# google/bayesnf

Hardware: AMD Instinct MI355X
Metric: train-steps/sec x ensemble_size (member-steps/s, whole job) (higher is better)
Workload: dtype bf16; 1 GPU; C2 chickenpox-like MAP: N=10232 rows, D=3, F=57, width=512, depth=2, NORMAL, full batch, lr=0.005; members_per_gpu=64, ensemble_size=64, parallelism=ensemble-shard x1 (no data-path collective)

## Files before the change

bayesnf_amd/csrc/bnf_api.hip:

```cpp
#include <hip/hip_runtime.h>
#include <cstring>
#include <rocprim/device/device_radix_sort.hpp>
#include <rocprim/device/device_segmented_radix_sort.hpp>

#include <dlfcn.h>

#include <atomic>
#include <cmath>
#include <cstdarg>
#include <cstdio>
#include <cstdlib>
#include <cstring>
#include <string>
#include <vector>

#include "../../include/bnf.h"
#include "bnf_gemm.h"
#include "bnf_kernels.h"
#include "bnf_panel.h"
#include "bnf_gemm8.h"
#include "bnf_sampling.h"
#include "bnf_extremes.h"
#include "bnf_episodes.h"
#include "bnf_scoring.h"
#include "bnf_rps.h"
#include "bnf_totals.h"
#include "bnf_dependence.h"
#include "bnf_ranking.h"
#include "bnf_stacking.h"

using namespace bnf;

static thread_local char g_err[512] = "";
static int fail(int code, const char* fmt, ...) {
  va_list ap;
  va_start(ap, fmt);
  vsnprintf(g_err, sizeof(g_err), fmt, ap);
  va_end(ap);
  return code;
}
#define HIPCHK(expr)                                                                   \
  do {                                                                                 \
    hipError_t _e = (expr);                                                            \
    if (_e != hipSuccess)                                                              \
      return fail(BNF_ERR_HIP, "%s failed: %s (%s:%d)", #expr, hipGetErrorString(_e), \
                  __FILE__, __LINE__);                                                 \
  } while (0)

enum KernelId {
  KID_PACK = 0, KID_FEAT, KID_FWD0, KID_FWD, KID_ROWLOSS, KID_LASTBWD, KID_DGRAD, KID_DGRAD0,
  KID_FEATBWD, KID_WGRAD0, KID_WGRAD, KID_ADAM, KID_VISAMPLE, KID_VIADAM, KID_FWDLAST, KID_PANEL, KID_COUNT
};
static const char* kKernelNames[KID_COUNT] = {
    "pack_weights", "featurize", "gemm_fwd_l0", "gemm_fwd", "row_loss", "last_bwd", "gemm_dgrad",
    "gemm_dgrad0", "feat_bwd", "gemm_wgrad_l0", "gemm_wgrad", "adam_map", "vi_sample", "vi_adam",
    "gemm_fwd_last", "panel_fwd_bwd"};

struct TimedLaunch {
  int kid;
  hipEvent_t t0, t1;
};

static constexpr int64_t kAtPad = 128;

struct bnf_handle {
  bnf_config cfg;
  NetDev nd;
  FreqTab ft;
  bool bf16 = false;
  int f32_split = 0;
  bool q8 = false;
  bool c8 = false;
  uint8_t* Wf8[BNF_MAX_LAYERS] = {}; uint8_t* Wb8[BNF_MAX_LAYERS] = {};
  uint8_t* H0q = nullptr;
  float* qscale = nullptr;
  int es = 4;
  int Ev = 0;
  int S = 1;
  int L = 0, W = 0, F = 0, Fp = 0, P = 0;
  int Wt = 0;
  bool pad = false;
  int64_t Pf = 0, Pp = 0;
  float* gradf = nullptr;
  float* theta_pad = nullptr;
  int32_t* pad_src = nullptr;
  int32_t* fold_src = nullptr;
  std::vector<int32_t> pad_src_h, fold_src_h;
  int32_t* fbmeta = nullptr;
  std::vector<int32_t> fbmeta_h;
  int fb_in_group = -1;
  int64_t N = 0, B = 0, Bp = 0;
  hipStream_t stream = nullptr;
  hipStream_t stream2 = nullptr;
  hipEvent_t ev_dz[BNF_MAX_LAYERS] = {};
  hipEvent_t ev_wg = nullptr;
  bool overlap = false;
  bool bound = false;
  int64_t adam_t = 0;
  float* params = nullptr;
  float* state = nullptr;
  char* ws = nullptr;
  const float* X = nullptr;
  const float* y = nullptr;
  float* theta_c = nullptr;
  float* grad = nullptr;
  float* stab = nullptr;
  float* stab_pred = nullptr;
  void* H0 = nullptr; void* H0t = nullptr;
  const float* ext_eps = nullptr;
  const uint32_t* vi_keys = nullptr; int64_t vi_key_rows = 0, vi_key_t0 = 0;
  const uint32_t* vi_draw_keys = nullptr; int64_t vi_draw_rows = 0;
  const int32_t* row_tab = nullptr; int64_t row_tab_epochs = 0, row_tab_e0 = 0;
  const uint32_t* row_keys = nullptr; int64_t row_keys_epochs = 0, row_keys_e0 = 0; int32_t row_key_rounds = 0;
  uint32_t* perm_bits[2] = {nullptr, nullptr}; int32_t* perm_val[2] = {nullptr, nullptr};
  unsigned* perm_seg = nullptr; void* perm_tmp = nullptr; size_t perm_tmp_bytes = 0;
  bool perm_ready = false;
  size_t owned_bytes = 0;
  int32_t* perm = nullptr; int64_t perm_epoch = -1;
  int32_t* leaf_off = nullptr; uint8_t* leaf_id = nullptr; int32_t n_leaves = 0;
  bool adam_clear_all = false;
  bool h0l = false;
  bool fold0 = false;
  void* A[BNF_MAX_LAYERS]; void* H[BNF_MAX_LAYERS]; void* Ht[BNF_MAX_LAYERS];
  void* dZ[BNF_MAX_LAYERS]; void* dZt[BNF_MAX_LAYERS];
  void* Kn[BNF_MAX_LAYERS]; void* Kt[BNF_MAX_LAYERS];
  int64_t pack_batch[BNF_MAX_LAYERS];
  float* dH0 = nullptr; float* out = nullptr; float* ybat = nullptr; float* loss_raw = nullptr;
  float* vacc = nullptr; float* dv = nullptr;
  bool vi_sample_pack = true, vi_keep_z = false;
  bool panel = false;
  void* Wf[BNF_MAX_LAYERS]; void* Wb[BNF_MAX_LAYERS];
  void* park[BNF_MAX_LAYERS];
    unsigned long long* prof_buf = nullptr;
  double prof_gap[16] = {0, 0, 0, 0, 0, 0, 0, 0, 0, 0, 0, 0, 0, 0, 0, 0};
  double prof_blocks = 0;
  int prof_threads = 0;
  bool recompute_a0 = false;
  bool fuse_last = false;
  int num_cus = 256;
  int tn_ring = 1;
  int skinny = 1;
  int big_tiles = 1;
  float* scal = nullptr;
  StepState* step_state = nullptr;
  hipGraphExec_t graph_exec = nullptr;
  int64_t graph_cols = 0;
  float* graph_losses = nullptr;
  int graph_mode = 0;
  float* qscratch = nullptr;
// ... 674 lines not shown
template <typename T>
static void run_pack_fragments(bnf_handle* h, const float* theta, int nmem) {
  LaunchScope ls(h, KID_PACK);
  int tiles = 0;
  const PackJobs jb = pack_jobs(h, &tiles);
  hipLaunchKernelGGL((k_pack_layers<T>), dim3((unsigned)tiles * (unsigned)nmem), dim3(256), 0, h->stream,
                     theta, (int64_t)h->Pf, jb, h->nd, h->scal);
}

template <int WN, int RT, bool H0L, bool DEEP, int CH, int FP, bool F0, bool C8 = false>
static void launch_panel_f(bnf_handle* h, const PanelArgs& pa) {
  constexpr int kLds = panel_lds_bytes(WN, RT, H0L, CH, FP);
  static_assert(kLds <= 160 * 1024, "LDS per workgroup");
  static std::atomic<uint64_t> attr_done{0};
  allow_lds(h, &k_panel_fwd_bwd<WN, RT, H0L, DEEP, CH, FP, F0, C8>, kLds, &attr_done);
  PanelArgs pa2 = pa;
  pa2.ablate = h->ablate;
  const unsigned blocks = (unsigned)(pa.members * pa.panels);
  {
    EpiArgs tmp{};
    phase_prof_begin(h, KID_PANEL, blocks, &tmp);
    pa2.prof = tmp.prof;
  }
  {
    LaunchScope ls(h, KID_PANEL);
    hipLaunchKernelGGL((k_panel_fwd_bwd<WN, RT, H0L, DEEP, CH, FP, F0, C8>), dim3(blocks), dim3(512), kLds, h->stream, pa2);
  }
  phase_prof_end(h, KID_PANEL, blocks, 512);
}
template <int WN, int RT, bool H0L, bool DEEP, int CH, int FP>
static void launch_panel_d(bnf_handle* h, const PanelArgs& pa) {
  if constexpr (H0L) {
    if (h->fold0) {
      if (pa.c8) {
        launch_panel_f<WN, RT, H0L, DEEP, CH, FP, true, true>(h, pa);
        return;
      }
      launch_panel_f<WN, RT, H0L, DEEP, CH, FP, true>(h, pa);
      return;
    }
  }
  launch_panel_f<WN, RT, H0L, DEEP, CH, FP, false>(h, pa);
}

template <int WN, int RT, bool H0L, int CH = 1, int FP = 64>
static void launch_panel(bnf_handle* h, const PanelArgs& pa) {
  if (pa.n_layers == 2) launch_panel_d<WN, RT, H0L, false, CH, FP>(h, pa);
  else launch_panel_d<WN, RT, H0L, true, CH, FP>(h, pa);
}

static void run_panel(bnf_handle* h, const float* theta, int nmem, const RowSrc& rs, float c,
                      const LossSink& sink, bool fragments_packed = false) {
  const int64_t Bp = h->Bp;
  if (!fragments_packed) run_pack_fragments<bf16_t>(h, theta, nmem);
  {
    LaunchScope ls(h, KID_FEAT);
    dim3 grid(cdiv(h->B, kFeatRows) * (unsigned)nmem);
    const size_t lds = (size_t)kFeatRows * (h->Fp + 8) * 2;
    static std::atomic<uint64_t> attr_done{0};
    allow_lds(h, &k_featurize<bf16_t>, 160 * 1024, &attr_done);
    hipLaunchKernelGGL((k_featurize<bf16_t>), grid, dim3(kFeatRows), lds, h->stream, h->nd, rs, h->X, h->stab,
                       h->y, h->scal, h->B, (bf16_t*)h->H0, Bp * h->Fp, (bf16_t*)h->H0t,
                       (int64_t)h->Fp * Bp, (int32_t)Bp, h->ybat, Bp, (int32_t)nmem, (int32_t)(h->fold0 ? 2 : 0), h->H0q);
  }
  bool feat_bwd_fused = false;
  PanelArgs pa{};
  pa.F = h->F; pa.Fp = h->Fp; pa.B = (int32_t)h->B; pa.members = nmem; pa.Wt = h->Wt;
  pa.theta = theta; pa.theta_stride = h->Pf; pa.scal = h->scal;
  const int L = h->L;
  pa.n_layers = L;
  for (int l = 0; l < L; ++l) {
    pa.off_bias[l] = h->nd.off_bias[l]; pa.off_ls[l] = h->nd.off_ls[l];
    pa.Wf[l] = (const bf16_t*)h->Wf[l]; pa.Wb[l] = (const bf16_t*)h->Wb[l];
    pa.Hout[l] = (bf16_t*)h->H[l]; pa.dZ[l] = (bf16_t*)h->dZ[l]; pa.park[l] = (bf16_t*)h->park[l];
  }
  pa.off_bias_out = h->nd.off_bias[L]; pa.off_ko = h->nd.off_kernel[L];
  pa.off_os = h->nd.off_os; pa.off_law = h->nd.off_law; pa.off_lns = h->nd.off_lns;
  pa.off_shape = h->nd.off_shape; pa.off_infl = h->nd.off_infl; pa.obs = h->nd.obs;
  pa.H0 = (const bf16_t*)h->H0t; pa.H0rm = (const bf16_t*)h->H0; pa.h0_batch = Bp * h->Fp;
  pa.w0_batch = h->pack_batch[0]; pa.w1_batch = h->pack_batch[1];
  pa.act_batch = Bp * h->W;
  pa.dH0t = h->dH0; pa.dh0_batch = (int64_t)h->Fp * Bp; pa.ldt = (int32_t)Bp;
  pa.ybat = h->ybat; pa.row_batch = Bp; pa.out = h->out; pa.out_batch = Bp;
  pa.grad = h->gradf; pa.grad_stride = h->Pf;
  pa.loss = sink.loss; pa.loss_raw = sink.raw; pa.loss_stride = sink.stride; pa.S = h->S;
  pa.loss_scale = sink.scale; pa.lik_c = c; pa.st = sink.st;
  pa.q8 = h->q8 ? 1 : 0; pa.qscale = h->qscale;
  pa.c8 = h->c8 ? 1 : 0; pa.w8_batch = (int64_t)h->W * h->W;
  for (int l = 0; l < L; ++l) { pa.Wf8[l] = h->Wf8[l]; pa.Wb8[l] = h->Wb8[l]; }
  auto with_fused_featbwd = [&]() {
    pa.fbmeta = h->fbmeta; pa.off_lsa = h->nd.off_lsa; pa.n_groups = h->nd.n_groups; pa.n_inputs = h->nd.D;
    pa.fb_in_group = h->fb_in_group;
    feat_bwd_fused = h->fbmeta != nullptr;
  };
  if (h->W == 1024) {
    pa.panels = (int32_t)(Bp / panel_rows(8, 2));
    if (h->h0l) {
      with_fused_featbwd();
      launch_panel<8, 2, true, 2>(h, pa);
    } else {
      launch_panel<8, 2, false, 2>(h, pa);
    }
  } else if (h->W == 512) {
    pa.panels = (int32_t)(Bp / panel_rows(8, 4));
    if (h->h0l) {
      with_fused_featbwd();
      launch_panel<8, 4, true>(h, pa);
    } else {
// ... 476 lines not shown
      return fail(BNF_ERR_INVALID, "fourier_degree[%d]", d);
    }
  }
  for (int k = 0; k < cfg->n_interact; ++k) {
    nd.interact[k][0] = cfg->interact[k][0];
    nd.interact[k][1] = cfg->interact[k][1];
  }
  nd.off_lns = cfg->off_log_noise_scale; nd.off_shape = cfg->off_shape; nd.off_infl = cfg->off_inflated;
  for (int l = 0; l <= h->L; ++l) {
    nd.off_bias[l] = cfg->off_bias[l];
    nd.off_kernel[l] = cfg->off_kernel[l];
  }
  h->Pf = h->P;
  if (h->pad) {
    const int W = h->W, Wt = h->Wt;
    int64_t pos = h->P;
    h->fold_src_h.resize((size_t)h->P);
    for (int64_t i = 0; i < h->P; ++i) h->fold_src_h[(size_t)i] = (int32_t)i;
    auto leaf = [&](int32_t off_true, int rows_t, int cols_t, int rows_p, int cols_p) {
      const int32_t off_pad = (int32_t)pos;
      for (int r = 0; r < rows_p; ++r)
        for (int c = 0; c < cols_p; ++c) {
          const bool in = r < rows_t && c < cols_t;
          const int32_t src = in ? off_true + r * cols_t + c : -1;
          h->pad_src_h.push_back(src);
          if (in) h->fold_src_h[(size_t)src] = (int32_t)pos;
          ++pos;
        }
      return off_pad;
    };
    for (int l = 0; l < h->L; ++l) {
      nd.off_bias[l] = leaf(cfg->off_bias[l], 1, Wt, 1, W);
      const int rt = (l == 0) ? h->F : Wt, rp = (l == 0) ? h->F : W;
      nd.off_kernel[l] = leaf(cfg->off_kernel[l], rt, Wt, rp, W);
    }
    nd.off_kernel[h->L] = leaf(cfg->off_kernel[h->L], Wt, 1, W, 1);
    while (pos % 4) { h->pad_src_h.push_back(-1); ++pos; }
    h->Pp = pos; h->Pf = pos;
  }
  for (int l = 0; l < h->L; ++l) nd.off_ls[l] = cfg->off_layer_scale[l];
  nd.off_os = cfg->off_output_scale; nd.off_lsa = cfg->off_lsa; nd.off_law = cfg->off_act_weight;
  h->ft.n = cfg->n_freqs;
  for (int j = 0; j < cfg->n_freqs; ++j) {
    h->ft.f[j] = cfg->freq[j];
    h->ft.h[j] = cfg->harmonic[j];
  }
  for (int k = 0; k < KID_COUNT; ++k) { h->acc_ms[k] = 0; h->acc_calls[k] = 0; }
  if (const char* ab = getenv("BNF_ABLATE")) h->ablate = atoi(ab);
  h->num_cus = prop.multiProcessorCount > 0 ? prop.multiProcessorCount : 256;
  if (const char* bt = getenv("BNF_BIG_TILES")) h->big_tiles = atoi(bt);
  if (const char* sk = getenv("BNF_WGRAD_SKINNY")) h->skinny = atoi(sk);
  if (const char* rg = getenv("BNF_TN_RING")) h->tn_ring = atoi(rg);
  if (const char* gm = getenv("BNF_GRAPH")) h->graph_mode = atoi(gm);
  h->adam_clear_all = getenv("BNF_ADAM_CLEAR_ALL") != nullptr;
  if (const char* v = getenv("BNF_VI_SAMPLE_PACK")) h->vi_sample_pack = atoi(v) != 0;
  if (const char* v = getenv("BNF_VI_KEEP_Z")) h->vi_keep_z = atoi(v) != 0;
  {
    int want = cfg->pipeline;
    if (const char* pf = getenv("BNF_PIPELINE")) want = atoi(pf);
    if (want != 0 && want != 1 && want != 3) {
      delete h;
      return fail(BNF_ERR_INVALID, "pipeline %d (0 auto, 1 layers, 3 panel)", want);
    }
    const bool can_panel = !cfg->forward_only && h->bf16 && h->L >= 2 && (h->W == 256 || h->W == 512 || h->W == 1024) && h->Fp <= 128;
    if (want == 3 && !can_panel) {
      delete h;
      return fail(BNF_ERR_INVALID, "panel pipeline needs a bf16 training handle with depth >= 2, width 256/512/1024 and <= 128 features");
    }
    h->panel = can_panel && (want == 3 || want == 0);
    if (h->q8 && !h->panel && !cfg->forward_only) {
      delete h;
      return fail(BNF_ERR_INVALID, "dtype fp8 (fp8 operand storage for the weight gradients) needs the row-panel pipeline: "
                  "depth >= 2, width 256 / 512 / 1024 after padding to 64, <= 128 padded features");
    }
    if (h->panel) h->Bp = align_up(h->B, 256);
    h->c8 = h->q8 && h->panel && !(getenv("BNF_FP8_CONTRACT") && atoi(getenv("BNF_FP8_CONTRACT")) == 0);
    const bool fl_ok = h->bf16 ? fused_last_supported<bf16_t>(h->W) : fused_last_supported<float>(h->W);
    h->fuse_last = !cfg->forward_only && !h->panel && want == 0 && fl_ok;
    h->recompute_a0 = !cfg->forward_only && !h->panel && want == 0 && h->L >= 2 && h->Fp <= 128;
  }
  h->h0l = panel_h0l(h);
  h->fold0 = h->h0l && h->F + 2 <= h->Fp && !(getenv("BNF_PANEL_FOLD0") && atoi(getenv("BNF_PANEL_FOLD0")) == 0);
  h->c8 = h->c8 && h->fold0;
  if (h->h0l &&
      !(getenv("BNF_PANEL_FEATBWD") && atoi(getenv("BNF_PANEL_FEATBWD")) == 0)) {
    int in_group = -1;
    for (int g = 0; g < cfg->n_groups; ++g)
      if (cfg->group_kind[g] == BNF_GROUP_INPUT) in_group = g;
    if (in_group >= 0) {
      std::vector<int32_t>& m = h->fbmeta_h;
      const int Fp = h->Fp;
      m.assign(Fp * 4 + BNF_MAX_GROUPS, 0);
      auto put = [&](int col, int kind, int g, int d1, int d2, int partner, int ucol, float coef) {
        m[4 * col] = kind | (g << 8) | (d1 << 16) | (d2 << 24);
        m[4 * col + 1] = partner | (ucol << 8);
        memcpy(&m[4 * col + 2], &coef, 4);
      };
      for (int c = 0; c < Fp; ++c) put(c, kFbNone, 0xff, 0xff, 0xff, 0, 0, 0.f);
      const int cin = cfg->group_col0[in_group];
      for (int g = 0; g < cfg->n_groups; ++g) {
        const int c0 = cfg->group_col0[g], nc = cfg->group_ncols[g];
        m[4 * Fp + g] = cfg->group_scale_off[g];
        switch (cfg->group_kind[g]) {
          case BNF_GROUP_INPUT:
            for (int d = 0; d < nc; ++d) put(c0 + d, kFbInput, g, d, 0xff, 0, 0, 0.f);
            break;
// ... 1292 lines not shown
```

bayesnf_amd/csrc/bnf_kernels.h:

```cpp
#pragma once

#include "bnf_device.h"
#include "../../include/bnf.h"

namespace bnf {

constexpr int kScalGroup = BNF_MAX_LAYERS + 2;
constexpr int kScalInput = kScalGroup + BNF_MAX_GROUPS;
constexpr int kScalGfac = kScalInput + BNF_MAX_INPUTS;
constexpr int kScalStride = kScalGfac + BNF_MAX_GROUPS;

__device__ __forceinline__ void sincos_rev(float x, float* s, float* c) {
  sincosf(6.28318530717958647692f * x, s, c);
}

struct NetDev {
  int32_t D, F, Fp, W, Wt, depth, P, n_groups, n_freqs, n_interact, obs;
  int32_t group_kind[BNF_MAX_GROUPS], group_arg[BNF_MAX_GROUPS], group_ncols[BNF_MAX_GROUPS],
      group_col0[BNF_MAX_GROUPS], group_scale_off[BNF_MAX_GROUPS];
  int32_t fdeg[BNF_MAX_INPUTS];
  float in_scale[BNF_MAX_INPUTS];
  int32_t interact[BNF_MAX_INTERACT][2];
  int32_t off_lns, off_shape, off_infl;
  int32_t off_bias[BNF_MAX_LAYERS + 1], off_kernel[BNF_MAX_LAYERS + 1], off_ls[BNF_MAX_LAYERS];
  int32_t off_os, off_lsa, off_law;
};

struct RowSrc {
  int32_t mode;
  int32_t S;
  uint64_t seed;
  uint64_t epoch;
  int64_t pos0;
  int64_t n_rows;
  int64_t member_offset;
  const int32_t* table;
  int64_t table_ld;
};

__device__ __forceinline__ int64_t row_of(const RowSrc& rs, int e, int64_t r) {
  if (rs.mode == 0) return r;
  if (rs.mode == 3) return (int64_t)rs.table[(int64_t)(e / rs.S) * rs.table_ld + rs.pos0 + r];
  if (rs.mode == 1) {
    const FeistelKey fk = feistel_key(rs.seed, (uint32_t)(rs.member_offset + e / rs.S), rs.epoch,
                                      STREAM_SHUFFLE, (uint64_t)rs.n_rows);
    return (int64_t)feistel_perm(fk, (uint64_t)(rs.pos0 + r));
  }
  const FeistelKey fk = feistel_key(rs.seed, 0u, rs.epoch, STREAM_VI_BATCH, (uint64_t)rs.n_rows);
  return (int64_t)feistel_perm(fk, (uint64_t)r);
}

constexpr float kTwoPiF = 6.2831854820251465f;

struct FreqTab {
  int32_t n;
  float f[BNF_MAX_FREQS], h[BNF_MAX_FREQS];
};

__global__ void k_seasonal_table(const float* __restrict__ X, int64_t n_rows, int D, FreqTab ft,
                                 float* __restrict__ S) {
  const int64_t r = (int64_t)blockIdx.x * blockDim.x + threadIdx.x;
  if (r >= n_rows) return;
  const float t = X[r * D];
  for (int j = 0; j < ft.n; ++j) {
    const float cf = kTwoPiF * ft.f[j];
    const float y = cf * t;
    double s, c;
    sincos((double)y, &s, &c);
    S[r * (2 * ft.n) + j] = (float)c / ft.h[j];
    S[r * (2 * ft.n) + ft.n + j] = (float)s / ft.h[j];
  }
}

constexpr int kFeatRows = 128;

template <typename T>
__global__ __launch_bounds__(kFeatRows) void k_featurize(
    NetDev nd, RowSrc rs, const float* __restrict__ X, const float* __restrict__ Stab,
    const float* __restrict__ y, const float* __restrict__ scal, int64_t B,
    T* __restrict__ H0, int64_t h0_batch, T* __restrict__ H0f, int64_t h0f_batch, int32_t ldt,
    float* __restrict__ ybat, int64_t ybat_batch, int32_t n_members, int32_t n_ones,
    uint8_t* __restrict__ H0q = nullptr) {
  extern __shared__ __attribute__((aligned(16))) char fsm[];
  constexpr int kEpc = 16 / Elem<T>::kBytes;
  T* tile = reinterpret_cast<T*>(fsm);
  const int pitch = nd.Fp + kEpc;
  const int e = (int)(blockIdx.x % (uint32_t)n_members);
  const int64_t r0 = (int64_t)(blockIdx.x / (uint32_t)n_members) * kFeatRows;
  const int64_t r = r0 + threadIdx.x;
  const float* sc = scal + (int64_t)e * kScalStride;
  if (r < B) {
    const int64_t row = row_of(rs, e, r);
    const float* x = X + row * nd.D;
    float xr[BNF_MAX_INPUTS], u[BNF_MAX_INPUTS];
#pragma unroll
    for (int d = 0; d < BNF_MAX_INPUTS; ++d) xr[d] = x[min(d, nd.D - 1)];
#pragma unroll
    for (int d = 0; d < BNF_MAX_INPUTS; ++d) u[d] = xr[d] / sc[kScalInput + min(d, nd.D - 1)];
    T* trow = tile + threadIdx.x * pitch;
    auto put = [&](int col, float v) { Elem<T>::store(trow + col, v); };
    for (int g = 0; g < nd.n_groups; ++g) {
      const float sp = sc[kScalGroup + g];
      const int c0 = nd.group_col0[g], nc = nd.group_ncols[g];
      const int kind = nd.group_kind[g];
      if (kind == BNF_GROUP_INPUT) {
        for (int d = 0; d < nd.D; ++d) put(c0 + d, u[d] * sp);
      } else if (kind == BNF_GROUP_FOURIER) {
        const int deg = nc >> 1;
        float ud = 0.f;
#pragma unroll
        for (int d = 0; d < BNF_MAX_INPUTS; ++d)
          if (d == nd.group_arg[g]) ud = u[d];
        for (int k = 0; k < deg; ++k) {
          float sn, cs;
          if constexpr (sizeof(T) == 2) {
            const float x = ud * (float)(1u << k);
            const float fx = x - floorf(x);
            sn = __builtin_amdgcn_sinf(fx);
            cs = __builtin_amdgcn_cosf(fx);
            const float q = __builtin_amdgcn_rcpf((float)(k + 1)) * sp;
            put(c0 + k, cs * q);
            put(c0 + deg + k, sn * q);
            continue;
          }
          sincos_rev(ud * (float)(1u << k), &sn, &cs);
          const float den = (float)(k + 1);
          put(c0 + k, (cs / den) * sp);
          put(c0 + deg + k, (sn / den) * sp);
        }
      } else if (kind == BNF_GROUP_SEASONAL) {
        const float* srow = Stab + row * nc;
        int j = 0;
        for (; j + 8 <= nc; j += 8) {
          float v[8];
#pragma unroll
          for (int q = 0; q < 8; ++q) v[q] = srow[j + q];
#pragma unroll
          for (int q = 0; q < 8; ++q) put(c0 + j + q, v[q] * sp);
        }
        for (; j < nc; ++j) put(c0 + j, srow[j] * sp);
      } else {
        for (int k = 0; k < nc; ++k) {
          float up = 0.f, uq = 0.f;
#pragma unroll
          for (int d = 0; d < BNF_MAX_INPUTS; ++d) {
            if (d == nd.interact[k][0]) up = u[d];
            if (d == nd.interact[k][1]) uq = u[d];
          }
          put(c0 + k, (up * uq) * sp);
        }
      }
    }
    for (int c = nd.F; c < nd.Fp; ++c) Elem<T>::store(trow + c, c < nd.F + n_ones ? 1.f : 0.f);
    if (ybat) ybat[(int64_t)e * ybat_batch + r] = y ? y[row] : 0.f;
  }
  __syncthreads();
  const int cpr = nd.Fp / kEpc;
  const int n_live = (int)min((int64_t)kFeatRows, B - r0);
  const int pitch_b = pitch * Elem<T>::kBytes;
  auto copy_out = [&](char* dst_block, int ppr, int sb, auto conv) {
    const int total = n_live * ppr;
    const int dc = kFeatRows % ppr, d_off = (kFeatRows / ppr) * pitch_b + dc * sb, wrap = pitch_b - ppr * sb;
    int cc = (int)threadIdx.x % ppr, off = ((int)threadIdx.x / ppr) * pitch_b + cc * sb;
    for (int q = threadIdx.x; q < total; q += 4 * kFeatRows) {
      u32x4 v[4];
      int offs[4];
#pragma unroll
      for (int i = 0; i < 4; ++i) {
        offs[i] = off;
        cc += dc; off += d_off;
        if (cc >= ppr) { cc -= ppr; off += wrap; }
      }
#pragma unroll
      for (int i = 0; i < 4; ++i)
        if (q + i * kFeatRows < total) v[i] = conv(fsm + offs[i]);
#pragma unroll
      for (int i = 0; i < 4; ++i)
        if (q + i * kFeatRows < total) *reinterpret_cast<u32x4*>(dst_block + (size_t)(q + i * kFeatRows) * 16) = v[i];
    }
  };
  if (n_live > 0) {
    copy_out(reinterpret_cast<char*>(H0 + (int64_t)e * h0_batch + r0 * nd.Fp), cpr, 16,
             [&](const char* src) { return *reinterpret_cast<const u32x4*>(src); });
  }
  if constexpr (sizeof(T) == 2) {
    if (H0q && n_live > 0) {
      __builtin_amdgcn_s_setreg(1 | (23 << 6), 1);
      copy_out(reinterpret_cast<char*>(H0q + (int64_t)e * h0_batch + r0 * nd.Fp), nd.Fp / 16, 32, [&](const char* src) {
        const u32x4 lo = *reinterpret_cast<const u32x4*>(src);
        const u32x4 hi = *reinterpret_cast<const u32x4*>(src + 16);
        return u32x4{bf16x4_to_fp8(lo[0], lo[1], 1.f), bf16x4_to_fp8(lo[2], lo[3], 1.f), bf16x4_to_fp8(hi[0], hi[1], 1.f),
                     bf16x4_to_fp8(hi[2], hi[3], 1.f)};
      });
    }
    if (H0f) {
      T* df = H0f + (int64_t)e * h0f_batch;
      const int ks0 = nd.Fp / 16;
      for (int q = threadIdx.x; q < kFeatRows * cpr; q += kFeatRows) {
        const int lr = q % kFeatRows, cc = q / kFeatRows;
        const int64_t rr = r0 + lr;
        if (rr < B)
          *reinterpret_cast<u32x4*>(df + ((((rr >> 5) * ks0 + (cc >> 1)) * 64 + (cc & 1) * 32 + (rr & 31)) << 3)) =
              *reinterpret_cast<const u32x4*>(tile + lr * pitch + cc * kEpc);
      }
    }
  }
  (void)ldt;
}

__global__ __launch_bounds__(256) void k_feat_bwd(
    NetDev nd, RowSrc rs, const float* __restrict__ X, const float* __restrict__ Stab,
    const float* __restrict__ theta, int64_t theta_stride, const float* __restrict__ scal, int64_t B,
    const float* __restrict__ dH0t, int64_t dh0_batch, int32_t ldt, float* __restrict__ grad,
    int64_t grad_stride) {
  __shared__ float red[4][BNF_MAX_GROUPS + BNF_MAX_INPUTS];
  const int e = blockIdx.y;
  const int64_t r = (int64_t)blockIdx.x * blockDim.x + threadIdx.x;
  const float* th = theta + (int64_t)e * theta_stride;
  const float* sc = scal + (int64_t)e * kScalStride;
  float dfs[BNF_MAX_GROUPS], dlsa[BNF_MAX_INPUTS];
#pragma unroll
  for (int g = 0; g < BNF_MAX_GROUPS; ++g) dfs[g] = 0.f;
#pragma unroll
  for (int d = 0; d < BNF_MAX_INPUTS; ++d) dlsa[d] = 0.f;
  if (r < B) {
    const int64_t row = row_of(rs, e, r);
    const float* x = X + row * nd.D;
    float xr[BNF_MAX_INPUTS], u[BNF_MAX_INPUTS], du[BNF_MAX_INPUTS];
#pragma unroll
    for (int d = 0; d < BNF_MAX_INPUTS; ++d) xr[d] = x[min(d, nd.D - 1)];
#pragma unroll
    for (int d = 0; d < BNF_MAX_INPUTS; ++d) {
      du[d] = 0.f;
      u[d] = d < nd.D ? xr[d] / sc[kScalInput + min(d, nd.D - 1)] : 0.f;
    }
    const float* dhp = dH0t + (int64_t)e * dh0_batch + r;
    auto dh = [&](int col) { return dhp[(int64_t)col * ldt]; };
#pragma unroll
    for (int g = 0; g < BNF_MAX_GROUPS; ++g) {
      if (g >= nd.n_groups) continue;
      const float sp = sc[kScalGroup + g];
      const int c0 = nd.group_col0[g], nc = nd.group_ncols[g];
      const int kind = nd.group_kind[g];
      float acc = 0.f;
      if (kind == BNF_GROUP_INPUT) {
#pragma unroll
        for (int d = 0; d < BNF_MAX_INPUTS; ++d)
          if (d < nd.D) {
            const float dhv = dh(c0 + d);
            acc += dhv * u[d];
            du[d] += sp * dhv;
          }
      } else if (kind == BNF_GROUP_FOURIER) {
        const int deg = nc >> 1;
        float ud = 0.f;
#pragma unroll
        for (int d = 0; d < BNF_MAX_INPUTS; ++d)
          if (d == nd.group_arg[g]) ud = u[d];
        float dud = 0.f;
// ... 32 lines not shown
          for (int q = 0; q < 8; ++q) acc += w[q] * v[q];
        }
        for (; j < nc; ++j) acc += dh(c0 + j) * srow[j];
      } else {
        for (int k = 0; k < nc; ++k) {
          const int p = nd.interact[k][0], q = nd.interact[k][1];
          float up = 0.f, uq = 0.f;
#pragma unroll
          for (int d = 0; d < BNF_MAX_INPUTS; ++d) {
            if (d == p) up = u[d];
            if (d == q) uq = u[d];
          }
          const float dhv = dh(c0 + k);
          acc += dhv * up * uq;
#pragma unroll
          for (int d = 0; d < BNF_MAX_INPUTS; ++d) {
            if (d == p) du[d] += sp * dhv * uq;
            if (d == q) du[d] += sp * dhv * up;
          }
        }
      }
      dfs[g] = acc;
    }
#pragma unroll
    for (int d = 0; d < BNF_MAX_INPUTS; ++d) dlsa[d] = -du[d] * u[d];
  }
  const int lane = threadIdx.x & 63, wave = threadIdx.x >> 6;
#pragma unroll
  for (int g = 0; g < BNF_MAX_GROUPS; ++g) {
    const float s = wave_sum(dfs[g]);
    if (lane == 0) red[wave][g] = s;
  }
#pragma unroll
  for (int d = 0; d < BNF_MAX_INPUTS; ++d) {
    const float s = wave_sum(dlsa[d]);
    if (lane == 0) red[wave][BNF_MAX_GROUPS + d] = s;
  }
  __syncthreads();
  float* gr = grad + (int64_t)e * grad_stride;
  const int t = threadIdx.x;
  if (t < nd.n_groups) {
    const float s = red[0][t] + red[1][t] + red[2][t] + red[3][t];
    atomicAdd(&gr[nd.group_scale_off[t]], sigmoidf(th[nd.group_scale_off[t]]) * s);
  } else if (t >= BNF_MAX_GROUPS && t < BNF_MAX_GROUPS + nd.D) {
    const float s = red[0][t] + red[1][t] + red[2][t] + red[3][t];
    atomicAdd(&gr[nd.off_lsa + (t - BNF_MAX_GROUPS)], s);
  }
}

__device__ __forceinline__ void member_scalars_row(const NetDev& nd, const float* __restrict__ th, float* __restrict__ o) {
  for (int l = 0; l < nd.depth; ++l) o[l] = softplusf(th[nd.off_ls[l]]);
  o[BNF_MAX_LAYERS] = sigmoidf(th[nd.off_law]);
  o[BNF_MAX_LAYERS + 1] = softplusf(th[nd.off_os]);
  for (int g = 0; g < nd.n_groups; ++g) o[kScalGroup + g] = softplusf(th[nd.group_scale_off[g]]);
  for (int d = 0; d < nd.D; ++d) o[kScalInput + d] = nd.in_scale[d] * expf(th[nd.off_lsa + d]);
  for (int g = 0; g < nd.n_groups; ++g) o[kScalGfac + g] = sigmoidf(th[nd.group_scale_off[g]]) / o[kScalGroup + g];
}
struct RowLossArgs {
  const float* theta;
  int64_t theta_stride;
  int64_t B;
  float* vacc;
  int64_t vacc_batch;
  const float* ybat;
  float* out;
  int64_t out_batch;
  float* dv;
  float* grad;
  int64_t grad_stride;
  float* loss;
  int64_t loss_stride;
  int32_t S;
  float loss_scale;
  float c;
  float* loss_raw;
  const StepState* st;
};

template <bool TRAIN>
__global__ __launch_bounds__(256) void k_row_loss(NetDev nd, RowLossArgs a) {
  __shared__ float s_red[4][5];
  const int e = blockIdx.y;
  const int64_t r = (int64_t)blockIdx.x * blockDim.x + threadIdx.x;
  const float* th = a.theta + (int64_t)e * a.theta_stride;
  const int L = nd.depth;
  const float gam_o = softplusf(th[nd.off_os]);
  float ll = 0.f, s_doutv = 0.f, s_dvsum = 0.f, s_par = 0.f, s_infl = 0.f;
  if (r < a.B) {
    const int64_t vi = (int64_t)e * a.vacc_batch + r;
    const float v = a.vacc[vi] * (1.0f / sqrtf((float)nd.Wt)) + th[nd.off_bias[L]];
    a.vacc[vi] = 0.f;
    const float out = gam_o * v;
    a.out[(int64_t)e * a.out_batch + r] = out;
    if constexpr (TRAIN) {
      const RowLoss rl = row_loss_eval(nd.obs, th, nd.off_lns, nd.off_shape, nd.off_infl, a.ybat[vi],
                                       out, a.c);
      ll = rl.ll; s_par = rl.d_par; s_infl = rl.d_infl;
      const float dout = rl.dout;
      s_doutv = dout * v;
      const float dvv = gam_o * dout;
      a.dv[vi] = dvv;
      s_dvsum = dvv;
    }
  }
  if constexpr (!TRAIN) return;
  const int lane = threadIdx.x & 63, wave = threadIdx.x >> 6;
  const float t0 = wave_sum(ll), t1 = wave_sum(s_doutv), t2 = wave_sum(s_dvsum), t3 = wave_sum(s_par);
  const float t4 = nd.obs == BNF_OBS_ZINB ? wave_sum(s_infl) : 0.f;
// ... 821 lines not shown
```

bayesnf_amd/csrc/bnf_panel.h:

```cpp
#pragma once

#include <type_traits>

#include "bnf_gemm.h"
#include "bnf_kernels.h"

namespace bnf {

struct PanelArgs {
  int32_t F, Fp, B, panels, members;
  int32_t Wt;
  const float* theta;
  int64_t theta_stride;
  const float* scal;
  int32_t n_layers;
  int32_t off_bias[BNF_MAX_LAYERS], off_ls[BNF_MAX_LAYERS];
  int32_t off_bias_out, off_ko, off_os, off_law;
  int32_t off_lns, off_shape, off_infl, obs;
  const bf16_t* H0;
  const bf16_t* H0rm;
  int64_t h0_batch;
  const bf16_t* Wf[BNF_MAX_LAYERS];
  const bf16_t* Wb[BNF_MAX_LAYERS];
  int64_t w0_batch, w1_batch;
// ... 57 lines not shown
  const int KSf = jb.n_pad[l] / 16, KSb = W / 16;
#pragma unroll
  for (int h = 0; h < 512 / NT; ++h) {
    const int q = tid + NT * h;
    const int frag = q >> 6, fl = q & 63;
    float v[8];
    {
      const int nl = (frag >> 2) * 32 + (fl & 31), kl = (frag & 3) * 16 + (fl >> 5) * 8;
#pragma unroll
      for (int j = 0; j < 8; ++j) v[j] = tile[kl + j][nl] * fs;
      if (fold && k0 + kl + 8 > jb.F0n && k0 + kl <= jb.F0n + 1) {
        const float gbv = fgb * th[jb.off_bias0 + n0 + nl];
        const float hi = Elem<bf16_t>::round(gbv);
#pragma unroll
        for (int j = 0; j < 8; ++j) {
          if (k0 + kl + j == jb.F0n) v[j] = hi;
          if (k0 + kl + j == jb.F0n + 1) v[j] = gbv - hi;
        }
      }
      const int64_t f = (int64_t)((n0 + nl) / 32) * KSf + (k0 + kl) / 16;
      store8(wf + (f * 64 + fl) * 8, v);
    }
    {
      const int il = (frag >> 2) * 32 + (fl & 31), cl = (frag & 3) * 16 + (fl >> 5) * 8;
#pragma unroll
      for (int j = 0; j < 8; ++j) v[j] = tile[il][cl + j];
      const int64_t f = (int64_t)((k0 + il) / 32) * KSb + (n0 + cl) / 16;
      store8(wb + (f * 64 + fl) * 8, v);
    }
  }
  if (jb.wf8[l] && l >= 1) {
    __builtin_amdgcn_s_setreg(1 | (23 << 6), 1);
    const int KS64 = W / 64;
    for (int q = tid; q < 512; q += NT) {
      const int lay = q >> 8, fr = (q >> 7) & 1, pc = (q >> 6) & 1, fl = q & 63;
      const int ml = fr * 32 + (fl & 31), kb = (fl >> 5) * 32 + pc * 16;
      uint32_t w4[4];
#pragma unroll
      for (int d = 0; d < 4; ++d) {
        float x[4];
#pragma unroll
        for (int b = 0; b < 4; ++b) x[b] = (lay == 0 ? tile[kb + 4 * d + b][ml] : tile[ml][kb + 4 * d + b]) * kW8Scale;
        int pk = __builtin_amdgcn_cvt_pk_fp8_f32(x[0], x[1], 0, false);
        pk = __builtin_amdgcn_cvt_pk_fp8_f32(x[2], x[3], pk, true);
        w4[d] = (uint32_t)pk;
      }
      uint8_t* base = (uint8_t*)(lay == 0 ? jb.wf8[l] : jb.wb8[l]) + e * jb.batch8;
      const int64_t f = lay == 0 ? (int64_t)((n0 + ml) / 32) * KS64 + k0 / 64 : (int64_t)((k0 + ml) / 32) * KS64 + n0 / 64;
      *reinterpret_cast<u32x4*>(base + f * 2048 + pc * 1024 + fl * 16) = u32x4{w4[0], w4[1], w4[2], w4[3]};
    }
  }
}
struct PackItem { int e, l, k0, n0; bool first; };
__device__ __forceinline__ PackItem pack_item_of(const PackJobs& jb) {
  const int n_tiles = jb.tile0[jb.n_layers];
  const uint32_t w = xcd_remap(blockIdx.x, gridDim.x);
  const int bx = (int)(w % (uint32_t)n_tiles);
  PackItem it;
  it.e = (int)(w / (uint32_t)n_tiles);
  int l = 0;
  while (l + 1 < jb.n_layers && bx >= jb.tile0[l + 1]) ++l;
  const int t = bx - jb.tile0[l], tn = jb.W / 64;
  it.l = l; it.k0 = (t / tn) * 64; it.n0 = (t % tn) * 64;
  it.first = bx == 0 && threadIdx.x == 0;
  return it;
}

template <typename T>
__global__ __launch_bounds__(256) void k_pack_layers(const float* __restrict__ theta, int64_t theta_stride,
                                                     PackJobs jb, NetDev nd, float* __restrict__ scal) {
  __shared__ float tile[64][65];
  const PackItem it = pack_item_of(jb);
  const float* th = theta + (int64_t)it.e * theta_stride;
  if (scal && it.first) member_scalars_row(nd, th, scal + (int64_t)it.e * kScalStride);
  const float* K = th + jb.off_kernel[it.l];
  const int tid = threadIdx.x;
#pragma unroll
  for (int i = 0; i < 4; ++i) {
    const int r = (tid >> 4) + 16 * i, c = (tid & 15) * 4;
    float v[4] = {0.f, 0.f, 0.f, 0.f};
    if (it.k0 + r < jb.n_in[it.l]) load4u(K + (int64_t)(it.k0 + r) * jb.W + it.n0 + c, 4, v);
#pragma unroll
    for (int j = 0; j < 4; ++j) tile[r][c + j] = v[j];
  }
  __syncthreads();
  pack_tile_fragments<T>(tile, jb, it.l, it.e, it.k0, it.n0, tid, th);
}

struct ViSampleArgs {
  const float* mu; const float* rho;
  int32_t P, S;
  uint64_t seed; int64_t member_offset; uint64_t step;
  float* z;
  int32_t write_z;
};
#ifndef BNF_VI_SP_THREADS
#define BNF_VI_SP_THREADS 512
#endif
template <typename T, int NT>
__global__ __launch_bounds__(NT) void k_vi_sample_pack(ViSampleArgs a, PackJobs jb, NetDev nd, float* __restrict__ scal) {
  constexpr int NI = 1024 / NT;
  __shared__ float tile[2][64][65];
  const PackItem it = pack_item_of(jb);
  const int e = it.e, l = it.l, tid = threadIdx.x;
  const int c = (tid & 15) * 4;
  float m[NI][4], sg[NI][4];
  int32_t pq[NI];
#pragma unroll
  for (int i = 0; i < NI; ++i) {
    const int r = (tid >> 4) + (NT / 16) * i;
    pq[i] = (it.k0 + r < jb.n_in[l]) ? jb.off_kernel[l] + (it.k0 + r) * jb.W + it.n0 + c : -1;
    if (pq[i] >= 0) {
      load4u(a.mu + (int64_t)e * a.P + pq[i], 4, m[i]);
      load4u(a.rho + (int64_t)e * a.P + pq[i], 4, sg[i]);
#pragma unroll
      for (int j = 0; j < 4; ++j) sg[i][j] = vi_sigma(sg[i][j]);
    }
  }
  for (int s = 0; s < a.S; ++s) {
    const int64_t en = (int64_t)e * a.S + s;
    float* zn = a.z + en * a.P;
    float (&tl)[64][65] = tile[s & 1];
    if (scal && it.first) member_scalars_row(nd, zn, scal + en * kScalStride);
#pragma unroll
    for (int i = 0; i < NI; ++i) {
      const int r = (tid >> 4) + (NT / 16) * i;
      float zv[4] = {0.f, 0.f, 0.f, 0.f};
      if (pq[i] >= 0) {
        const Normal4 n = vi_eps_quad(a.seed, (uint32_t)(a.member_offset + e), (uint32_t)s,
                                      (uint32_t)(pq[i] + kEpsQuadPhase) >> 2, a.step, STREAM_VI_EPS);
#pragma unroll
        for (int j = 0; j < 4; ++j) zv[j] = m[i][j] + sg[i][j] * n.v[j];
        if (a.write_z) store4u(zn + pq[i], 4, zv);
      }
#pragma unroll
      for (int j = 0; j < 4; ++j) tl[r][c + j] = zv[j];
    }
    __syncthreads();
    pack_tile_fragments<T, NT>(tl, jb, l, en, it.k0, it.n0, tid, zn);
  }
}

#ifndef BNF_EPI_FENCE_EVERY
#define BNF_EPI_FENCE_EVERY 1
#endif
#ifndef BNF_PANEL_PD
#define BNF_PANEL_PD 4
#endif
constexpr int kPanelPD = BNF_PANEL_PD;
constexpr int kAuxNT = 2;

__host__ __device__ constexpr int panel_rows(int wn, int rt) { return 32 * rt * (8 / wn); }
__host__ __device__ constexpr int panel_lds_bytes(int wn, int rt, bool h0l, int ch = 1, int fp = 64) {
  const int W = 64 * wn * ch, BM = panel_rows(wn, rt), RB = 8 / wn;
  const int image = BM * (W * 2 + 16), dots = 8 * 64 * 36 * 4;
  const bool own_fb = fp > 64 || RB > 1 || W < 512;
// ... 1403 lines not shown
```

Measured before the change: 36820 member-steps/s.

## Merge weight packing and featurization into a single prep-step launch

```diff
diff --git a/bayesnf_amd/csrc/bnf_api.hip b/bayesnf_amd/csrc/bnf_api.hip
--- a/bayesnf_amd/csrc/bnf_api.hip
+++ b/bayesnf_amd/csrc/bnf_api.hip
@@ -49,12 +49,12 @@
 
 enum KernelId {
   KID_PACK = 0, KID_FEAT, KID_FWD0, KID_FWD, KID_ROWLOSS, KID_LASTBWD, KID_DGRAD, KID_DGRAD0,
-  KID_FEATBWD, KID_WGRAD0, KID_WGRAD, KID_ADAM, KID_VISAMPLE, KID_VIADAM, KID_FWDLAST, KID_PANEL, KID_COUNT
+  KID_FEATBWD, KID_WGRAD0, KID_WGRAD, KID_ADAM, KID_VISAMPLE, KID_VIADAM, KID_FWDLAST, KID_PANEL, KID_PREP, KID_COUNT
 };
 static const char* kKernelNames[KID_COUNT] = {
     "pack_weights", "featurize", "gemm_fwd_l0", "gemm_fwd", "row_loss", "last_bwd", "gemm_dgrad",
     "gemm_dgrad0", "feat_bwd", "gemm_wgrad_l0", "gemm_wgrad", "adam_map", "vi_sample", "vi_adam",
-    "gemm_fwd_last", "panel_fwd_bwd"};
+    "gemm_fwd_last", "panel_fwd_bwd", "prep_step"};
 
 struct TimedLaunch {
   int kid;
@@ -95,6 +95,7 @@
   hipEvent_t ev_dz[BNF_MAX_LAYERS] = {};
   hipEvent_t ev_wg = nullptr;
   bool overlap = false;
+  bool merge_prep = true;
   bool bound = false;
   int64_t adam_t = 0;
   float* params = nullptr;
@@ -875,8 +876,21 @@
 static void run_panel(bnf_handle* h, const float* theta, int nmem, const RowSrc& rs, float c,
                       const LossSink& sink, bool fragments_packed = false) {
   const int64_t Bp = h->Bp;
-  if (!fragments_packed) run_pack_fragments<bf16_t>(h, theta, nmem);
-  {
+  if (!fragments_packed && h->merge_prep) {
+    LaunchScope ls(h, KID_PREP);
+    int tiles = 0;
+    const PackJobs jb = pack_jobs(h, &tiles);
+    FeatJob fj{};
+    fj.rs = rs; fj.X = h->X; fj.Stab = h->stab; fj.y = h->y; fj.B = h->B;
+    fj.H0 = (bf16_t*)h->H0; fj.h0_batch = Bp * h->Fp; fj.H0f = (bf16_t*)h->H0t; fj.h0f_batch = (int64_t)h->Fp * Bp;
+    fj.ybat = h->ybat; fj.ybat_batch = Bp; fj.n_members = nmem; fj.n_ones = h->fold0 ? 2 : 0; fj.H0q = h->H0q;
+    const PrepGrid pg = prep_grid((uint32_t)tiles * (uint32_t)nmem, cdiv(h->B, kPrepFeatRows) * (uint32_t)nmem);
+    static std::atomic<uint64_t> attr_done{0};
+    allow_lds(h, &k_prep_step<bf16_t>, 160 * 1024, &attr_done);
+    hipLaunchKernelGGL((k_prep_step<bf16_t>), dim3(8u * (pg.groups_pack + pg.groups_feat)), dim3(256),
+                       (size_t)prep_step_lds(h->Fp), h->stream, theta, (int64_t)h->Pf, jb, h->nd, h->scal, fj, pg);
+  } else {
+    if (!fragments_packed) run_pack_fragments<bf16_t>(h, theta, nmem);
     LaunchScope ls(h, KID_FEAT);
     dim3 grid(cdiv(h->B, kFeatRows) * (unsigned)nmem);
     const size_t lds = (size_t)kFeatRows * (h->Fp + 8) * 2;
@@ -1459,6 +1473,7 @@
   if (const char* sk = getenv("BNF_WGRAD_SKINNY")) h->skinny = atoi(sk);
   if (const char* rg = getenv("BNF_TN_RING")) h->tn_ring = atoi(rg);
   if (const char* gm = getenv("BNF_GRAPH")) h->graph_mode = atoi(gm);
+  if (const char* ml = getenv("BNF_MERGED_LAUNCHES")) h->merge_prep = atoi(ml) != 0;
   h->adam_clear_all = getenv("BNF_ADAM_CLEAR_ALL") != nullptr;
   if (const char* v = getenv("BNF_VI_SAMPLE_PACK")) h->vi_sample_pack = atoi(v) != 0;
   if (const char* v = getenv("BNF_VI_KEEP_Z")) h->vi_keep_z = atoi(v) != 0;
diff --git a/bayesnf_amd/csrc/bnf_kernels.h b/bayesnf_amd/csrc/bnf_kernels.h
--- a/bayesnf_amd/csrc/bnf_kernels.h
+++ b/bayesnf_amd/csrc/bnf_kernels.h
@@ -74,27 +74,37 @@
 
 constexpr int kFeatRows = 128;
 
-template <typename T>
-__global__ __launch_bounds__(kFeatRows) void k_featurize(
-    NetDev nd, RowSrc rs, const float* __restrict__ X, const float* __restrict__ Stab,
-    const float* __restrict__ y, const float* __restrict__ scal, int64_t B,
-    T* __restrict__ H0, int64_t h0_batch, T* __restrict__ H0f, int64_t h0f_batch, int32_t ldt,
-    float* __restrict__ ybat, int64_t ybat_batch, int32_t n_members, int32_t n_ones,
-    uint8_t* __restrict__ H0q = nullptr) {
-  extern __shared__ __attribute__((aligned(16))) char fsm[];
+__device__ __forceinline__ float feat_group_scale(const NetDev& nd, const float* __restrict__ th, int g) {
+  return softplusf(th[nd.group_scale_off[g]]);
+}
+__device__ __forceinline__ float feat_input_scale(const NetDev& nd, const float* __restrict__ th, int d) {
+  return nd.in_scale[d] * expf(th[nd.off_lsa + d]);
+}
+
+template <typename T, int FR, int NT, typename Ready>
+__device__ __forceinline__ void featurize_rows(
+    const NetDev& nd, const RowSrc& rs, const float* __restrict__ X, const float* __restrict__ Stab,
+    const float* __restrict__ y, const float* sc, int64_t B,
+    T* __restrict__ H0, int64_t h0_batch, T* __restrict__ H0f, int64_t h0f_batch,
+    float* __restrict__ ybat, int64_t ybat_batch, int32_t n_ones, uint8_t* __restrict__ H0q,
+    int e, int64_t r0, char* fsm, Ready scales_ready) {
+  static_assert(NT >= FR, "one thread per row");
   constexpr int kEpc = 16 / Elem<T>::kBytes;
   T* tile = reinterpret_cast<T*>(fsm);
   const int pitch = nd.Fp + kEpc;
-  const int e = (int)(blockIdx.x % (uint32_t)n_members);
-  const int64_t r0 = (int64_t)(blockIdx.x / (uint32_t)n_members) * kFeatRows;
   const int64_t r = r0 + threadIdx.x;
-  const float* sc = scal + (int64_t)e * kScalStride;
-  if (r < B) {
-    const int64_t row = row_of(rs, e, r);
+  const bool live = (NT == FR || (int)threadIdx.x < FR) && r < B;
+  int64_t row = 0;
+  float xr[BNF_MAX_INPUTS] = {};
+  if (live) {
+    row = row_of(rs, e, r);
     const float* x = X + row * nd.D;
-    float xr[BNF_MAX_INPUTS], u[BNF_MAX_INPUTS];
 #pragma unroll
     for (int d = 0; d < BNF_MAX_INPUTS; ++d) xr[d] = x[min(d, nd.D - 1)];
+  }
+  scales_ready();
+  if (live) {
+    float u[BNF_MAX_INPUTS];
 #pragma unroll
     for (int d = 0; d < BNF_MAX_INPUTS; ++d) u[d] = xr[d] / sc[kScalInput + min(d, nd.D - 1)];
     T* trow = tile + threadIdx.x * pitch;
@@ -156,13 +166,13 @@
   }
   __syncthreads();
   const int cpr = nd.Fp / kEpc;
-  const int n_live = (int)min((int64_t)kFeatRows, B - r0);
+  const int n_live = (int)min((int64_t)FR, B - r0);
   const int pitch_b = pitch * Elem<T>::kBytes;
   auto copy_out = [&](char* dst_block, int ppr, int sb, auto conv) {
     const int total = n_live * ppr;
-    const int dc = kFeatRows % ppr, d_off = (kFeatRows / ppr) * pitch_b + dc * sb, wrap = pitch_b - ppr * sb;
+    const int dc = NT % ppr, d_off = (NT / ppr) * pitch_b + dc * sb, wrap = pitch_b - ppr * sb;
     int cc = (int)threadIdx.x % ppr, off = ((int)threadIdx.x / ppr) * pitch_b + cc * sb;
-    for (int q = threadIdx.x; q < total; q += 4 * kFeatRows) {
+    for (int q = threadIdx.x; q < total; q += 4 * NT) {
       u32x4 v[4];
       int offs[4];
 #pragma unroll
@@ -173,10 +183,10 @@
       }
 #pragma unroll
       for (int i = 0; i < 4; ++i)
-        if (q + i * kFeatRows < total) v[i] = conv(fsm + offs[i]);
+        if (q + i * NT < total) v[i] = conv(fsm + offs[i]);
 #pragma unroll
       for (int i = 0; i < 4; ++i)
-        if (q + i * kFeatRows < total) *reinterpret_cast<u32x4*>(dst_block + (size_t)(q + i * kFeatRows) * 16) = v[i];
+        if (q + i * NT < total) *reinterpret_cast<u32x4*>(dst_block + (size_t)(q + i * NT) * 16) = v[i];
     }
   };
   if (n_live > 0) {
@@ -196,8 +206,8 @@
     if (H0f) {
       T* df = H0f + (int64_t)e * h0f_batch;
       const int ks0 = nd.Fp / 16;
-      for (int q = threadIdx.x; q < kFeatRows * cpr; q += kFeatRows) {
-        const int lr = q % kFeatRows, cc = q / kFeatRows;
+      for (int q = threadIdx.x; q < FR * cpr; q += NT) {
+        const int lr = q % FR, cc = q / FR;
         const int64_t rr = r0 + lr;
         if (rr < B)
           *reinterpret_cast<u32x4*>(df + ((((rr >> 5) * ks0 + (cc >> 1)) * 64 + (cc & 1) * 32 + (rr & 31)) << 3)) =
@@ -205,6 +215,20 @@
       }
     }
   }
+}
+
+template <typename T>
+__global__ __launch_bounds__(kFeatRows) void k_featurize(
+    NetDev nd, RowSrc rs, const float* __restrict__ X, const float* __restrict__ Stab,
+    const float* __restrict__ y, const float* __restrict__ scal, int64_t B,
+    T* __restrict__ H0, int64_t h0_batch, T* __restrict__ H0f, int64_t h0f_batch, int32_t ldt,
+    float* __restrict__ ybat, int64_t ybat_batch, int32_t n_members, int32_t n_ones,
+    uint8_t* __restrict__ H0q = nullptr) {
+  extern __shared__ __attribute__((aligned(16))) char fsm[];
+  const int e = (int)(blockIdx.x % (uint32_t)n_members);
+  const int64_t r0 = (int64_t)(blockIdx.x / (uint32_t)n_members) * kFeatRows;
+  featurize_rows<T, kFeatRows, kFeatRows>(nd, rs, X, Stab, y, scal + (int64_t)e * kScalStride, B, H0, h0_batch, H0f,
+                                          h0f_batch, ybat, ybat_batch, n_ones, H0q, e, r0, fsm, [] {});
   (void)ldt;
 }
 
@@ -343,8 +367,8 @@
   for (int l = 0; l < nd.depth; ++l) o[l] = softplusf(th[nd.off_ls[l]]);
   o[BNF_MAX_LAYERS] = sigmoidf(th[nd.off_law]);
   o[BNF_MAX_LAYERS + 1] = softplusf(th[nd.off_os]);
-  for (int g = 0; g < nd.n_groups; ++g) o[kScalGroup + g] = softplusf(th[nd.group_scale_off[g]]);
-  for (int d = 0; d < nd.D; ++d) o[kScalInput + d] = nd.in_scale[d] * expf(th[nd.off_lsa + d]);
+  for (int g = 0; g < nd.n_groups; ++g) o[kScalGroup + g] = feat_group_scale(nd, th, g);
+  for (int d = 0; d < nd.D; ++d) o[kScalInput + d] = feat_input_scale(nd, th, d);
   for (int g = 0; g < nd.n_groups; ++g) o[kScalGfac + g] = sigmoidf(th[nd.group_scale_off[g]]) / o[kScalGroup + g];
 }
 struct RowLossArgs {
diff --git a/bayesnf_amd/csrc/bnf_panel.h b/bayesnf_amd/csrc/bnf_panel.h
--- a/bayesnf_amd/csrc/bnf_panel.h
+++ b/bayesnf_amd/csrc/bnf_panel.h
@@ -133,9 +133,9 @@
   }
 }
 struct PackItem { int e, l, k0, n0; bool first; };
-__device__ __forceinline__ PackItem pack_item_of(const PackJobs& jb) {
+__device__ __forceinline__ PackItem pack_item_of(const PackJobs& jb, uint32_t b, uint32_t count) {
   const int n_tiles = jb.tile0[jb.n_layers];
-  const uint32_t w = xcd_remap(blockIdx.x, gridDim.x);
+  const uint32_t w = xcd_remap(b, count);
   const int bx = (int)(w % (uint32_t)n_tiles);
   PackItem it;
   it.e = (int)(w / (uint32_t)n_tiles);
@@ -148,10 +148,9 @@
 }
 
 template <typename T>
-__global__ __launch_bounds__(256) void k_pack_layers(const float* __restrict__ theta, int64_t theta_stride,
-                                                     PackJobs jb, NetDev nd, float* __restrict__ scal) {
-  __shared__ float tile[64][65];
-  const PackItem it = pack_item_of(jb);
+__device__ __forceinline__ void pack_layers_block(float (&tile)[64][65], const float* __restrict__ theta, int64_t theta_stride,
+                                                  const PackJobs& jb, const NetDev& nd, float* __restrict__ scal,
+                                                  const PackItem& it) {
   const float* th = theta + (int64_t)it.e * theta_stride;
   if (scal && it.first) member_scalars_row(nd, th, scal + (int64_t)it.e * kScalStride);
   const float* K = th + jb.off_kernel[it.l];
@@ -166,6 +165,64 @@
   }
   __syncthreads();
   pack_tile_fragments<T>(tile, jb, it.l, it.e, it.k0, it.n0, tid, th);
+}
+template <typename T>
+__global__ __launch_bounds__(256) void k_pack_layers(const float* __restrict__ theta, int64_t theta_stride,
+                                                     PackJobs jb, NetDev nd, float* __restrict__ scal) {
+  __shared__ float tile[64][65];
+  pack_layers_block<T>(tile, theta, theta_stride, jb, nd, scal, pack_item_of(jb, blockIdx.x, gridDim.x));
+}
+
+#ifndef BNF_PREP_FEAT_ROWS
+#define BNF_PREP_FEAT_ROWS 128
+#endif
+constexpr int kPrepFeatRows = BNF_PREP_FEAT_ROWS;
+struct FeatJob {
+  RowSrc rs;
+  const float* X; const float* Stab; const float* y;
+  int64_t B;
+  bf16_t* H0; int64_t h0_batch;
+  bf16_t* H0f; int64_t h0f_batch;
+  float* ybat; int64_t ybat_batch;
+  int32_t n_members, n_ones;
+  uint8_t* H0q;
+};
+__host__ __device__ constexpr int prep_feat_tile_bytes(int Fp) { return kPrepFeatRows * (Fp + 8) * 2; }
+__host__ __device__ constexpr int prep_step_lds(int Fp) {
+  const int feat = prep_feat_tile_bytes(Fp) + kScalStride * 4, pack = 64 * 65 * 4;
+  return feat > pack ? feat : pack;
+}
+struct PrepGrid { uint32_t n_pack, n_feat, groups_pack, groups_feat; };
+__host__ __device__ inline PrepGrid prep_grid(uint32_t n_pack, uint32_t n_feat) {
+  return {n_pack, n_feat, (n_pack + 7u) / 8u, (n_feat + 7u) / 8u};
+}
+template <typename T>
+__global__ __launch_bounds__(256, 8) void k_prep_step(const float* __restrict__ theta, int64_t theta_stride, PackJobs jb,
+                                                   NetDev nd, float* __restrict__ scal, FeatJob fj, PrepGrid pg) {
+  extern __shared__ __attribute__((aligned(16))) char psm[];
+  const uint32_t grp = blockIdx.x >> 3, x = blockIdx.x & 7u, groups = pg.groups_pack + pg.groups_feat;
+  const uint32_t f0 = (uint32_t)((uint64_t)grp * pg.groups_feat / groups);
+  const uint32_t f1 = (uint32_t)((uint64_t)(grp + 1) * pg.groups_feat / groups);
+  if (f1 == f0) {
+    const uint32_t b = (grp - f0) * 8u + x;
+    if (b >= pg.n_pack) return;
+    pack_layers_block<T>(*reinterpret_cast<float (*)[64][65]>(psm), theta, theta_stride, jb, nd, scal,
+                         pack_item_of(jb, b, pg.n_pack));
+    return;
+  }
+  const uint32_t b = f0 * 8u + x;
+  if (b >= pg.n_feat) return;
+  const int e = (int)(b % (uint32_t)fj.n_members);
+  const int64_t r0 = (int64_t)(b / (uint32_t)fj.n_members) * kPrepFeatRows;
+  float* sc = reinterpret_cast<float*>(psm + prep_feat_tile_bytes(nd.Fp));
+  const float* th = theta + (int64_t)e * theta_stride;
+  featurize_rows<T, kPrepFeatRows, 256>(nd, fj.rs, fj.X, fj.Stab, fj.y, sc, fj.B, fj.H0, fj.h0_batch, fj.H0f, fj.h0f_batch,
+                                        fj.ybat, fj.ybat_batch, fj.n_ones, fj.H0q, e, r0, psm, [&] {
+    const int t = 255 - (int)threadIdx.x;
+    if (t < nd.n_groups) sc[kScalGroup + t] = feat_group_scale(nd, th, t);
+    else if (t >= BNF_MAX_GROUPS && t < BNF_MAX_GROUPS + nd.D) sc[kScalInput + t - BNF_MAX_GROUPS] = feat_input_scale(nd, th, t - BNF_MAX_GROUPS);
+    __syncthreads();
+  });
 }
 
 struct ViSampleArgs {
@@ -182,7 +239,7 @@
 __global__ __launch_bounds__(NT) void k_vi_sample_pack(ViSampleArgs a, PackJobs jb, NetDev nd, float* __restrict__ scal) {
   constexpr int NI = 1024 / NT;
   __shared__ float tile[2][64][65];
-  const PackItem it = pack_item_of(jb);
+  const PackItem it = pack_item_of(jb, blockIdx.x, gridDim.x);
   const int e = it.e, l = it.l, tid = threadIdx.x;
   const int c = (tid & 15) * 4;
   float m[NI][4], sg[NI][4];
```

Measured after the change: 37140 member-steps/s, median of 6. Within noise of the previous version (+0.9%).
